# vgl-hub/teloscope

Hardware: AMD Instinct MI355X
Metric: Gbases/s scanned (whole node), 3 Gb FASTA TTAGGG w=1000 s=500 (higher is better)
Workload: dtype u8; 1 GPU; configs[1]: synthetic 3.00 Gb / 200 contigs, -c TTAGGG -p TTAGGG,TCAGGG,TGAGGG,TTGGGG -x 1 -w 1000 -s 500 -r -g -e -m -i, 124 patterns k=6; bases=3000000000, windows=6000095, matches=91510666, tiles=260970

## Files before the change

teloscope_amd/csrc/kernels.hip:

```cpp
#include <hip/hip_runtime.h>
#include <stdint.h>

#include <type_traits>

#include "ts_device.h"
#include "ts_internal.h"

#define set_prio(p) __builtin_amdgcn_s_setprio(p)
constexpr int kPrioPass = 3;
constexpr int kPrioAppend = 2;
constexpr int kPrioWindows = 2;

namespace {

typedef unsigned long long u64;
#define LDS __attribute__((address_space(3)))
typedef uint32_t u32x2 __attribute__((ext_vector_type(2)));
typedef LDS unsigned char lds_u8;
typedef LDS uint16_t lds_u16;
typedef LDS uint32_t lds_u32;

__device__ __forceinline__ lds_u16 *lds_at16(uint32_t addr) { return (lds_u16 *)(uintptr_t)addr; }
__device__ __forceinline__ lds_u8 *lds_at8(uint32_t addr) { return (lds_u8 *)(uintptr_t)addr; }

__host__ __device__ inline uint32_t align16(uint32_t x) { return (x + 15u) & ~15u; }

struct SliceLayout { uint32_t codes, rec, wacc, stage, park, bytes; };

__host__ __device__ inline SliceLayout slice_layout(const TsScanParams &P) {
    SliceLayout s;
    uint32_t o = 0;
    s.codes = o; o += align16((P.nch * 63u + 1u) * 8u);
    s.rec = o; o += (P.windows_on && P.nuc_on) ? align16((P.max_windows + P.halo_blocks) * 16u) : 0u;
    s.wacc = o; o += P.windows_on ? align16((P.max_windows + (P.acc_blocks ? P.halo_blocks : 0u)) * 8u * (P.acc_copies + (P.acc_blocks ? 1u : 0u))) : 0u;
    s.stage = o; o += (P.stage_cap + 64u) * (P.stage_u16 ? 2u : 4u);
    s.park = o; o += 32u;
    s.bytes = o;
    return s;
}

__host__ __device__ inline uint32_t queue_region(const TsScanParams &P) {
    const uint32_t a = TS_LIST * 2u;
    return (P.table_rows * 4u + P.fc_bytes + a - 1u) & ~(a - 1u);
}

__host__ __device__ inline uint32_t lds_total(const TsScanParams &P) {
    return queue_region(P) + P.waves_per_wg * (TS_LIST * 2u + slice_layout(P).bytes);
}

template <bool FC_BYTES, bool PAIR_BYTES, int WAVES_EU, bool EMIT, bool FAST>
__global__ __launch_bounds__(TS_MAX_WG_THREADS, WAVES_EU)
void ts_scan_tiles(const TsScanParams P) {
    const bool st16 = FAST ? true : P.stage_u16 != 0u;
    const bool accb = FAST ? true : P.acc_blocks != 0u;
    extern __shared__ __attribute__((aligned(16))) unsigned char lds_raw[];
    const uint32_t tid = threadIdx.x;
    const uint32_t lane = tid & 63u;
    const uint32_t wave = (uint32_t)__builtin_amdgcn_readfirstlane((int)(tid >> 6));

    const uint32_t table_bytes = P.table_rows * 4u + P.fc_bytes;
    {
        const uint4 *src = (const uint4 *)P.table;
        uint4 *dst = (uint4 *)lds_raw;
        const uint32_t n16 = table_bytes >> 4;
        for (uint32_t i = tid; i < n16; i += blockDim.x) dst[i] = src[i];
    }
    __syncthreads();

    const SliceLayout SL = slice_layout(P);
    lds_u8 *lds = (lds_u8 *)lds_raw;
    uint32_t qbase = queue_region(P) + wave * (TS_LIST * 2u);
    uint32_t qmask = TS_LIST * 2u - 2u;
    asm volatile("" : "+v"(qbase));
    asm volatile("" : "+s"(qmask));
    lds_u8 *slice = lds + queue_region(P) + P.waves_per_wg * (TS_LIST * 2u) + wave * SL.bytes;
    lds_u32 *codes = (lds_u32 *)(slice + SL.codes);
    lds_u32 *rec = (lds_u32 *)(slice + SL.rec);
    lds_u32 *stage = (lds_u32 *)(slice + SL.stage);
    LDS u64 *wacc = (LDS u64 *)(slice + SL.wacc);
    lds_u32 *park = (lds_u32 *)(slice + SL.park);
    const uint32_t acc_rows = P.max_windows + (accb ? P.halo_blocks : 0u);
    const uint32_t acc_off = (lane & (P.acc_copies - 1u)) * acc_rows;

    const uint32_t k = P.k;
    const uint32_t rowbits = 2u * (k + 1u) - 4u;
    const uint32_t kmask = (1u << (2u * k)) - 1u;
    const uint32_t pmask = (1u << (2u * (k + 1u))) - 1u;
    const lds_u32 *fc_table = (const lds_u32 *)(lds + P.table_rows * 4u);
    const lds_u8 *fc_bytes = (const lds_u8 *)fc_table;
    const uint32_t tab_base = (uint32_t)(uintptr_t)lds;
    if (PAIR_BYTES && (tab_base & pmask) != 0u) __builtin_trap();

    const uint32_t total_waves = gridDim.x * P.waves_per_wg;
    const uint32_t gw = blockIdx.x * P.waves_per_wg + wave;
    typedef const TsScanParams __attribute__((address_space(4))) *KernArgs;
    auto tail_params = [&]() -> KernArgs {
        KernArgs q = (KernArgs)__builtin_amdgcn_kernarg_segment_ptr();
        asm volatile("" : "+s"(q));
        return q;
    };
    uint32_t cursor = 0;
    if (EMIT) { park[4] = 0u; park[5] = 0u; }
    const uint32_t nwper = P.halo_blocks + 1u;

    typedef const TsTile __attribute__((address_space(4))) *ConstTiles;
    const ConstTiles const_tiles = (ConstTiles)(uintptr_t)P.tiles;
    uint4 n0 = make_uint4(0, 0, 0, 0), n1 = n0;
    uint32_t ticket = 0;
    const uint32_t ngroups = P.dynamic_tiles ? P.ticket_groups : 1u;
    const uint32_t group = blockIdx.x % ngroups;
    const uint32_t group_waves = ((gridDim.x - group + ngroups - 1u) / ngroups) * P.waves_per_wg;
    auto take_ticket = [&](KernArgs Q) -> uint32_t {
        const u64 a = (u64)(uintptr_t)(Q->tile_tickets + (Q->ticket_slot * Q->ticket_groups + group) * TS_TICKET_STRIDE);
        uint32_t lo = (uint32_t)a, hi = (uint32_t)(a >> 32);
        asm volatile("" : "+v"(lo), "+v"(hi));
        typedef __attribute__((address_space(1))) uint32_t *GlobalU32;
        return __hip_atomic_fetch_add((GlobalU32)(uintptr_t)(((u64)hi << 32) | lo), 1u, __ATOMIC_RELAXED, __HIP_MEMORY_SCOPE_AGENT);
    };
    if (P.dynamic_tiles && gw == 0 && lane < ngroups) P.tile_tickets[((1u - P.ticket_slot) * ngroups + lane) * TS_TICKET_STRIDE] = 0u;
    const uint32_t first_tile = P.dynamic_tiles ? group + ngroups * ((blockIdx.x / ngroups) * P.waves_per_wg + wave) : gw;
    if (first_tile < P.ntiles) {
        if (P.dynamic_tiles && lane == 0) ticket = take_ticket(tail_params());
        const unsigned char *ls = P.in + (const_tiles[first_tile].in_off & ~15ull) + lane * 32u;
        n0 = *(const uint4 *)ls; n1 = *(const uint4 *)(ls + 16);
    }
    for (uint32_t tile = first_tile, tile_next = 0; tile < P.ntiles; tile = tile_next) {
        struct { u64 in_off; uint32_t nrel, nwin, own_len; } T;
        {
            const ConstTiles q = const_tiles + tile;
            uint32_t lo = (uint32_t)q->in_off, hi = (uint32_t)(q->in_off >> 32), a = q->nrel, b = q->nwin, c = q->own_len;
            asm volatile("" : "+s"(lo), "+s"(hi), "+s"(a), "+s"(b), "+s"(c));
            T.in_off = ((u64)hi << 32) | lo; T.nrel = a; T.nwin = b; T.own_len = c;
        }
        const uint32_t sh = (uint32_t)(T.in_off & 15ull);
        const unsigned char *src = P.in + (T.in_off - sh);
        const uint32_t nblk = T.nwin + P.halo_blocks;
        const uint32_t span = nblk * P.s;
        const uint32_t xend = sh + T.nrel;
        uint32_t need = sh + (T.nrel < span + 16u ? T.nrel : span + 16u);
        uint32_t nch = (need + 16u + TS_CHUNK - 1u) / TS_CHUNK;
        if (nch > P.nch) nch = P.nch;
        nch = (uint32_t)__builtin_amdgcn_readfirstlane((int)nch);
        bool has_invalid = false;
        const uint32_t own_end = sh + T.own_len;
        uint32_t done = 0, ccan = 0, cfwd = 0;
        uint32_t flushed = 0;
        auto stage_at = [&](uint32_t i) -> uint32_t { return st16 ? (uint32_t)((lds_u16 *)stage)[i] : stage[i]; };
        auto flush_stage = [&]() {
            __builtin_amdgcn_wave_barrier();
            const uint32_t n = done - flushed;
            KernArgs Q = tail_params();
            const uint32_t cap = Q->region_cap;
            uint32_t *const wave_out = Q->matches_out + (u64)gw * cap;
            const bool rec16 = Q->rec16 != 0u;
            for (uint32_t i = lane; i < n; i += 64u) {
                const uint32_t o = cursor + flushed + i;
                if (o < cap) {
                    if (rec16) gstore_lo16((uint16_t *)Q->matches_out + (u64)gw * cap + o, stage_at(i));
                    else gstore(wave_out + o, stage_at(i));
                }
            }
            if (EMIT) park[5] = 1u;
            __builtin_amdgcn_s_waitcnt(0x0F70);
            __builtin_amdgcn_wave_barrier();
            flushed = done;
        };
        uint32_t tile_vis = 0;
        auto finish_records = [&]() {
            __builtin_amdgcn_wave_barrier();
            KernArgs Q = tail_params();
            const uint32_t cap = Q->region_cap;
            uint32_t *const wave_out = Q->matches_out + (u64)gw * cap;
            uint32_t ln = lane;
            asm volatile("" : "+v"(ln));
            uint32_t n = done - flushed;
            bool redo = false;
            if (EMIT) redo = __builtin_amdgcn_readfirstlane((int)park[5]) != 0;
            const bool rec16 = Q->rec16 != 0u;
            uint16_t *const wave_out16 = (uint16_t *)Q->matches_out + (u64)gw * cap;
            if (!EMIT || redo) {
                if (!EMIT && st16 && rec16 && cursor + flushed + n <= cap) {
                    const uint32_t n4 = n & ~3u;
                    uint16_t *const dst = wave_out16 + cursor + flushed;
                    for (uint32_t i = 4u * ln; i < n4; i += 256u) {
                        const u32x2 q = *(const LDS u32x2 *)((lds_u16 *)stage + i);
                        gstore_unaligned((unsigned char *)(dst + i), (u64)q.x | ((u64)q.y << 32));
                    }
                    if (ln < n - n4) gstore_lo16(dst + n4 + ln, stage_at(n4 + ln));
                } else
                for (uint32_t i = ln; i < n; i += 64u) {
                    const uint32_t o = cursor + flushed + i;
                    if (o < cap) {
                        if (rec16) gstore_lo16(wave_out16 + o, stage_at(i));
                        else gstore(wave_out + o, stage_at(i));
                    }
                }
                flushed = done;
                if (!EMIT) return;
                asm volatile("s_waitcnt vmcnt(0)" ::: "memory");
                park[5] = 0u;
                n = done;
            }
            const uint32_t base = redo ? 0u : flushed;
            uint32_t ch_first = 0, ch_last = 0, ch_cc = 0, ch_w1 = 0, vout = 0;
            const uint32_t vbase = (uint32_t)__builtin_amdgcn_readfirstlane((int)park[4]);
            typedef const uint32_t __attribute__((address_space(4))) *ConstU32;
            const uint32_t zone = ((ConstU32)(uintptr_t)Q->tile_zone)[tile];
            const uint32_t vis_cap = Q->vis_cap;
            const bool wide = FAST ? false : Q->vis_wide != 0u;
            void *const vis_out = Q->vis_out;
            const u64 vwave = (u64)gw * vis_cap;
            const uint32_t kdist = P.kdist;
            const bool rec_fit = cursor + base + n <= cap, vis_fit = vbase + n <= vis_cap;
            auto look = [&](const uint32_t r, const uint32_t nrow, const uint32_t i0, auto full_row) {
                constexpr bool FULL = decltype(full_row)::value;
                const uint32_t u = r >> 2;
                const u64 live_m = FULL ? ~0ull : low_bits(nrow);
                const u64 canm = ballot64((r & 1u) != 0u);
                if (i0 == 0u) ch_first = (uint32_t)__builtin_amdgcn_readfirstlane((int)u);
                {
                    u64 vm = canm;
                    if (zone != TS_ZONE_NONE) vm = live_m & (canm | ballot64(u < (zone & 0xFFFFu)) | ballot64(u >= (zone >> 16)));
                    if (vm != 0ull) {
                        const uint32_t at = vbase + vout + __builtin_amdgcn_mbcnt_hi((uint32_t)(vm >> 32), __builtin_amdgcn_mbcnt_lo((uint32_t)vm, 0u));
                        if (__builtin_amdgcn_inverse_ballot_w64(vm) && (vis_fit || at < vis_cap)) {
                            if (wide) gstore((uint32_t *)vis_out + (vwave + at), r);
                            else gstore((uint16_t *)vis_out + (vwave + at), (uint16_t)r);
                        }
                        vout += (uint32_t)__popcll(vm);
                    }
                }
                const uint32_t ncan = (uint32_t)__popcll(canm);
                const uint32_t t = ch_cc + ncan;
                if ((t | (~ch_w1 & TS_CHAIN_HEADS)) != 0u) {
                    const uint32_t below = lane_below(u, ch_last);
                    const u64 H = FULL ? ballot64(u - below > kdist) : live_m & ballot64(u - below > kdist);
                    if (__builtin_expect(t >= 4u, 0)) {
                        if (H != 0ull) {
                            const u64 ahead = ~H & (H - 1ull);
                            const uint32_t top_head = 63u - (uint32_t)__builtin_clzll(H);
                            const u64 below_top = low_bits(top_head);
                            const uint32_t carry = ch_cc + (uint32_t)__popcll(canm & ahead);
                            if (!(ch_w1 & TS_CHAIN_HEADS)) ch_w1 |= carry < 0x7FFFu ? carry : 0x7FFFu;
                            else if (carry >= 4u) ch_w1 |= TS_CHAIN_INNER;
                            if (__popcll(canm & ~ahead & below_top) >= 4) {
                                const u64 above = ln < 63u ? H >> (ln + 1u) : 0ull;
                                const uint32_t next = above ? ln + 1u + (uint32_t)__builtin_ctzll(above) : 64u;
                                const bool mine4 = __popcll(canm & low_bits(next) & ~low_bits(ln)) >= 4;
                                if (ballot64(((H >> ln) & 1ull) && ln != top_head && mine4) != 0ull) ch_w1 |= TS_CHAIN_INNER;
                            }
                            ch_w1 |= TS_CHAIN_HEADS;
                            ch_cc = (uint32_t)__popcll(canm & ~below_top);
                        } else {
                            ch_cc = t;
                        }
                    } else {
                        uint32_t tmp;
                        u64 m;
                        asm volatile("s_bitcmp1_b32 %[w1], 15\n\t"
                                     "s_cbranch_scc1 .Lts_cq%=\n\t"
                                     "s_cmp_eq_u64 %[H], 0\n\t"
                                     "s_cbranch_scc1 .Lts_cq%=\n\t"
                                     "s_ff1_i32_b64 %[tmp], %[H]\n\t"
                                     "s_lshl_b64 %[m], -1, %[tmp]\n\t"
                                     "s_andn2_b64 %[m], %[canm], %[m]\n\t"
                                     "s_bcnt1_i32_b64 %[tmp], %[m]\n\t"
                                     "s_add_i32 %[tmp], %[tmp], %[cc]\n\t"
                                     "s_or_b32 %[w1], %[w1], %[tmp]\n\t"
                                     "s_bitset1_b32 %[w1], 15\n"
                                     ".Lts_cq%=:\n\t"
                                     "s_flbit_i32_b64 %[tmp], %[H]\n\t"
                                     "s_xor_b32 %[tmp], %[tmp], 63\n\t"
                                     "s_lshl_b64 %[m], -1, %[tmp]\n\t"
                                     "s_and_b64 %[m], %[m], %[canm]\n\t"
                                     "s_bcnt1_i32_b64 %[tmp], %[m]\n\t"
                                     "s_cmp_lg_u64 %[H], 0\n\t"
                                     "s_cselect_b32 %[cc], %[tmp], %[t]"
                                     : [cc] "+s"(ch_cc), [w1] "+s"(ch_w1), [tmp] "=&s"(tmp), [m] "=&s"(m)
                                     : [H] "s"(H), [canm] "s"(canm), [t] "s"(t)
                                     : "scc");
                    }
                }
                ch_last = (uint32_t)__builtin_amdgcn_readlane((int)u, FULL ? 63 : (int)nrow - 1);
            };
            if (!redo) {
                const uint32_t nfull = n & ~63u;
                for (uint32_t i0 = 0; i0 < nfull; i0 += 64u) {
                    const uint32_t o = cursor + base + i0 + ln;
                    const uint32_t r = stage_at(i0 + ln);
                    auto put = [&]() { if (rec16) gstore_lo16(wave_out16 + o, r); else gstore(wave_out + o, r); };
                    if (rec_fit) put();
                    else if (o < cap) put();
                    look(r, 64u, i0, std::true_type{});
                }
                for (uint32_t i0 = nfull; i0 < n; i0 += 64u) {
                    const uint32_t nrow = n - i0 < 64u ? n - i0 : 64u;
                    const uint32_t o = cursor + base + i0 + ln;
                    uint32_t r = 0u;
                    if (ln < nrow) {
                        r = stage_at(i0 + ln);
                        if (o < cap) {
                            if (rec16) gstore_lo16(wave_out16 + o, r);
                            else gstore(wave_out + o, r);
                        }
                    }
                    look(r, nrow, i0, std::false_type{});
                }
            } else {
                for (uint32_t i0 = 0; i0 < n; i0 += 64u) {
                    const uint32_t nrow = n - i0 < 64u ? n - i0 : 64u;
                    const uint32_t o = cursor + base + i0 + ln;
                    uint32_t r = 0u;
                    if (ln < nrow && o < cap)
                        r = rec16 ? (uint32_t)__hip_atomic_load(wave_out16 + o, __ATOMIC_RELAXED, __HIP_MEMORY_SCOPE_AGENT)
                                  : __hip_atomic_load(wave_out + o, __ATOMIC_RELAXED, __HIP_MEMORY_SCOPE_AGENT);
                    look(r, nrow, i0, std::false_type{});
                }
            }
            flushed = done;
            const uint32_t z15 = ch_cc < 0x7FFFu ? ch_cc : 0x7FFFu;
            if (!(ch_w1 & TS_CHAIN_HEADS)) ch_w1 |= z15;
            const u64 voff = vwave + vbase;
            if (ln == 0u) gstore((uint4 *)&Q->tile_chain[4ull * tile], make_uint4((ch_first & 0xFFFFu) | (ch_last << 16), ch_w1 | (z15 << 16), (uint32_t)voff, (uint32_t)(voff >> 32)));
            tile_vis = vout;
            park[4] = vbase + vout;
        };
        if (P.windows_on)
            for (uint32_t it = lane; it < acc_rows * 2u * (P.acc_copies + (accb ? 1u : 0u)); it += 64u) ((lds_u32 *)wacc)[it] = 0u;

        uint32_t qhead = 0, qcount = 0;
        auto drain_queue = [&](const uint32_t threshold) {
            if (qcount >= threshold && qcount > 0u) set_prio(kPrioPass);
            while (qcount >= threshold && qcount > 0u) {
                const uint32_t n = qcount < 64u ? qcount : 64u;
                if (done - flushed + 64u > P.stage_cap) flush_stage();
                const bool live = lane < n;
                const uint32_t xp = live ? (uint32_t)*lds_at16(((qhead + lane * 2u) & qmask) | qbase) : 0u;
                const lds_u32 *cw = codes + __builtin_amdgcn_ubfe(xp, 4, 12);
                const uint32_t kw = __builtin_amdgcn_alignbit(cw[1], cw[0], (xp & 15u) * 2u);
                const uint32_t idx = kw & kmask;
                uint32_t fc;
                if (PAIR_BYTES) fc = __builtin_amdgcn_ubfe((uint32_t)*lds_at8(kw & pmask), 2, 2);
                else if (FC_BYTES) fc = fc_bytes[idx];
                else fc = (fc_table[idx >> 4] >> ((idx & 15u) << 1)) & 3u;
                const uint32_t u = xp - sh;
                uint32_t q = 0u, o = u;
                if (P.windows_on) {
                    uint32_t qs;
                    if (P.div_exact) {
                        q = __umul24(u, P.s_magic22) >> 22; qs = __umul24(q, P.s);
                    } else {
                        q = __umul24(u, P.s_inv) >> 16; qs = __umul24(q, P.s);
                        if (qs > u) { --q; qs -= P.s; }
                    }
                    o = u - qs;
                }
                u64 valid_m = low_bits(n) & ballot64(xp >= sh);
                if (P.straddle_fix) valid_m &= ~ballot64(o + k > P.s);
                const u64 bal = valid_m & ballot64(xp < own_end);
                const bool valid = __builtin_amdgcn_inverse_ballot_w64(valid_m), owned = __builtin_amdgcn_inverse_ballot_w64(bal);
                const uint32_t rank = __builtin_amdgcn_mbcnt_hi((uint32_t)(bal >> 32), __builtin_amdgcn_mbcnt_lo((uint32_t)bal, 0u));
                const uint32_t slot = owned ? (done - flushed) + rank : P.stage_cap + lane;
                const uint32_t record = (u << 2) | fc;
                if (st16) ((lds_u16 *)stage)[slot] = (uint16_t)record; else stage[slot] = record;
                done += (uint32_t)__popcll(bal);
                const u64 can_all = ballot64((fc & 1u) != 0u), fwd_all = ballot64((fc & 2u) != 0u);
                const bool is_can = __builtin_amdgcn_inverse_ballot_w64(can_all), is_fwd = __builtin_amdgcn_inverse_ballot_w64(fwd_all);
                const u64 canm = can_all & bal;
                ccan += (uint32_t)__popcll(canm);
                cfwd += (uint32_t)__popcll(fwd_all & bal);
                const u64 inc = (u64)(is_can ? 1u : 0x10000u) | ((u64)(is_fwd ? 1u : 0x10000u) << 32);
                if (P.windows_on && accb) {
                    if (valid && q < nblk) atomicAdd((unsigned long long *)(wacc + acc_off + q), inc);
                    const u64 over = valid_m & ballot64(o + k > P.s);
                    if (over != 0ull) {
                        if (__builtin_amdgcn_inverse_ballot_w64(over) && q < nblk) atomicAdd((unsigned long long *)(wacc + P.acc_copies * acc_rows + q), inc);
                    }
                } else if (P.windows_on) {
                    for (uint32_t j = 0; j < nwper; ++j) {
                        const uint32_t wi = q - j;
                        const bool in = valid && wi < T.nwin && o + k + j * P.s <= P.w;
                        if (in) atomicAdd((unsigned long long *)(wacc + acc_off + wi), inc);
                    }
                }
                qhead = (qhead + 2u * n) & (TS_LIST * 2u - 1u);
                qcount -= n;
            }
            set_prio(0);
            __builtin_amdgcn_wave_barrier();
        };

        auto scan_chunk = [&](const uint32_t cpos, const uint32_t ch, const uint4 v0, const uint4 v1) -> uint32_t {
            const uint32_t x[8] = {v0.x, v0.y, v0.z, v0.w, v1.x, v1.y, v1.z, v1.w};
            uint32_t t[8], e[8], bad = 0;
#pragma unroll
            for (int i = 0; i < 8; ++i) {
                t[i] = x[i] & 0x06060606u;
                e[i] = __builtin_amdgcn_perm(0xFF47FF54u, 0xFF43FF41u, t[i]);
                bad = __builtin_amdgcn_bitop3_b32(x[i], e[i], bad, 0xBE);
            }
            uint32_t wa = pack16(t), wb = pack16(t + 4);

            const uint32_t pos0 = cpos + lane * 32u;
            uint32_t inv = 0;
            const bool slow = __any((bad & P.fold_mask) != 0u) || (cpos + 2048u > xend);
            if (slow) {
                asm volatile("; non-ACGT bases or segment end in this chunk" ::: "memory");
                uint32_t b4[8];
#pragma unroll
                for (int i = 0; i < 8; ++i) {
                    const uint32_t d = (x[i] & P.fold_mask) ^ e[i];
                    const uint32_t nz = ((((d & 0x7F7F7F7Fu) + 0x7F7F7F7Fu) | d) & 0x80808080u) >> 7;
                    b4[i] = __builtin_amdgcn_udot4(nz, 0x08040201u, 0u, false);
                }
                inv = b4[0] | (b4[1] << 4) | (b4[2] << 8) | (b4[3] << 12) |
                      (b4[4] << 16) | (b4[5] << 20) | (b4[6] << 24) | (b4[7] << 28);
                uint32_t inside = inv;
                if (pos0 < sh) inside &= ~0u << (sh - pos0);
                if (pos0 + 32u > xend) {
                    const uint32_t nv = xend > pos0 ? xend - pos0 : 0u;
                    inside &= ~(~0u << nv);
                    inv |= ~0u << nv;
                }
                if (__any(inside != 0u)) has_invalid = true;
                wa = pack16(t); wb = pack16(t + 4);
            }

            const uint32_t nx = (uint32_t)__builtin_amdgcn_mov_dpp((int)wa, 0x130, 0xf, 0xf, false);

            uint32_t tmp[16], ent[16];
            const uint32_t xa = PAIR_BYTES ? __builtin_amdgcn_alignbit(wb, wa, 16) : 0u;
            const uint32_t xb = PAIR_BYTES ? __builtin_amdgcn_alignbit(nx, wb, 16) : 0u;
#pragma unroll
            for (int j = 0; j < 16; ++j) {
                if (PAIR_BYTES) {
                    tmp[j] = 0;
                    const uint32_t word = (j & 7) <= 4 ? (j < 8 ? wa : wb) : (j < 8 ? xa : xb);
                    const uint32_t bit = (j & 7) <= 4 ? 4 * (j & 7) : 4 * ((j & 7) - 4);
                    const uint32_t addr = __builtin_amdgcn_ubfe(word, bit, 2u * (k + 1u)) | tab_base;
                    asm volatile("ds_read_u8 %0, %1" : "=v"(ent[j]) : "v"(addr));
                    continue;
                }
                if (j < 8) tmp[j] = (j == 0) ? wa : __builtin_amdgcn_alignbit(wb, wa, 4 * j);
                else tmp[j] = (j == 8) ? wb : __builtin_amdgcn_alignbit(nx, wb, 4 * (j - 8));
                {
                    const uint32_t row = __builtin_amdgcn_ubfe(tmp[j], 4, rowbits);
                    const uint32_t addr = tab_base + (row << 2);
                    asm volatile("ds_read_b32 %0, %1" : "=v"(ent[j]) : "v"(addr));
                }
            }
            const uint32_t h = ch + lane;
            *(LDS u32x2 *)(codes + 2u * h) = (u32x2){wa, wb};

            uint32_t M32 = 0;
            asm volatile("s_waitcnt lgkmcnt(0)" ::: "memory");
            __builtin_amdgcn_sched_barrier(0);
#pragma unroll
            for (int j = 0; j < 16; ++j)
                M32 = __builtin_amdgcn_alignbit(PAIR_BYTES ? ent[j] : ent[j] >> ((tmp[j] << 1) & 31u), M32, 2);

            if (slow) {
                const uint32_t inv_next = (uint32_t)__builtin_amdgcn_mov_dpp((int)inv, 0x130, 0xf, 0xf, false);
                const u64 iv = (u64)inv | ((u64)inv_next << 32);
                uint32_t kb = 0;
                for (uint32_t i = 0; i < k; ++i) kb |= (uint32_t)(iv >> i);
                M32 &= ~kb;
            }

            if (lane == 63u) M32 = 0;
            return M32;
        };
        auto append_chunk = [&](const uint32_t M32, const uint32_t cpos, const uint32_t nm0, const uint32_t incl0, const uint32_t total0) {
            const uint32_t lbase = cpos + lane * 32u;
            constexpr uint32_t kGroup = TS_LIST / 32u;
            const bool dense = TS_LIST < TS_CHUNK && total0 > TS_LIST;
            const uint32_t ngroups = dense ? 64u / kGroup : 1u;
            for (uint32_t gi = 0; gi < ngroups; ++gi) {
                uint32_t m = M32, nm = nm0, incl = incl0, total = total0;
                if (dense) {
                    m = (lane / kGroup == gi) ? M32 : 0u;
                    nm = __popc(m);
                    incl = wave_scan_add(nm);
                    total = (uint32_t)__builtin_amdgcn_readlane((int)incl, 63);
                }
                drain_queue(qcount + total > TS_LIST ? 1u : 64u);
                uint32_t o = qhead + 2u * (qcount + incl - nm);
                while (m) {
                    *lds_at16((o & qmask) | qbase) = (uint16_t)(lbase + (uint32_t)__builtin_ctz(m));
                    o += 2u;
                    m &= m - 1u;
                }
                qcount += total;
                __builtin_amdgcn_wave_barrier();
            }
        };
        auto append_pair = [&](const uint32_t mA, const uint32_t cposA, const uint32_t mB, const uint32_t cposB) {
            if (!__any((mA | mB) != 0u)) return;
            set_prio(kPrioAppend);
            const uint32_t nA = __popc(mA), nB = __popc(mB);
            const uint32_t incl = wave_scan_add(nA | (nB << 16));
            const uint32_t tot = (uint32_t)__builtin_amdgcn_readlane((int)incl, 63);
            const uint32_t totA = tot & 0xFFFFu, totB = tot >> 16;
            if (totA + totB + 63u > TS_LIST) {
                asm volatile("; dense pair of chunks" ::: "memory");
                if (totA) append_chunk(mA, cposA, nA, incl & 0xFFFFu, totA);
                if (totB) append_chunk(mB, cposB, nB, incl >> 16, totB);
                set_prio(0);
                return;
            }
            drain_queue(64u);
            set_prio(kPrioAppend);
            uint32_t o = qhead + 2u * (qcount + (incl & 0xFFFFu) - nA), m = mA;
            uint32_t lbase = cposA + lane * 32u;
            while (m) {
                *lds_at16((o & qmask) | qbase) = (uint16_t)(lbase + (uint32_t)__builtin_ctz(m));
                o += 2u;
                m &= m - 1u;
            }
            o = qhead + 2u * (qcount + totA + (incl >> 16) - nB); m = mB;
            lbase = cposB + lane * 32u;
            while (m) {
                *lds_at16((o & qmask) | qbase) = (uint16_t)(lbase + (uint32_t)__builtin_ctz(m));
                o += 2u;
                m &= m - 1u;
            }
            qcount += totA + totB;
            set_prio(0);
            __builtin_amdgcn_wave_barrier();
        };
        {
            const uint32_t last_pos = (uint32_t)__builtin_amdgcn_readfirstlane((int)((nch - 1u) * TS_CHUNK));
            const unsigned char *lsrc = src + lane * 32u;
            uint4 a0 = n0, a1 = n1, b0, b1;
            uint32_t cpos = 0, ch = 0;
            for (uint32_t c = 0; c < nch; c += 2u) {
                const uint32_t p1 = cpos + TS_CHUNK < last_pos ? cpos + TS_CHUNK : last_pos;
                b0 = *(const uint4 *)(lsrc + p1);
                b1 = *(const uint4 *)(lsrc + p1 + 16);
                __builtin_amdgcn_sched_barrier(0);
                const uint32_t mA = scan_chunk(cpos, ch, a0, a1);
                uint32_t mB = 0u;
                const bool pair = c + 1u < nch;
                if (pair) {
                    const uint32_t p2 = cpos + 2u * TS_CHUNK < last_pos ? cpos + 2u * TS_CHUNK : last_pos;
                    a0 = *(const uint4 *)(lsrc + p2);
                    a1 = *(const uint4 *)(lsrc + p2 + 16);
                    __builtin_amdgcn_sched_barrier(0);
                    mB = scan_chunk(cpos + TS_CHUNK, ch + 63u, b0, b1);
                }
                append_pair(mA, cpos, mB, cpos + TS_CHUNK);
                cpos += 2u * TS_CHUNK; ch += 126u;
            }
        }
#define TS_REQUEST_NEXT_TILE()                                                                                                   \
        {                                                                                                                        \
                           \
            __builtin_amdgcn_s_waitcnt(0x0F70);                                                                                  \
            KernArgs Q = tail_params();                                                                                          \
            const bool dyn = Q->dynamic_tiles != 0u;                                                                             \
            tile_next = dyn ? group + Q->ticket_groups * (group_waves + (uint32_t)__builtin_amdgcn_readfirstlane((int)ticket))   \
                            : tile + total_waves;                                                                                \
            if (tile_next < P.ntiles) {                       \
                const unsigned char *ls = P.in + (const_tiles[tile_next].in_off & ~15ull) + lane * 32u;                          \
                n0 = *(const uint4 *)ls; n1 = *(const uint4 *)(ls + 16);                                                         \
                if (dyn && lane == 0) ticket = take_ticket(Q);                         \
            }                                                                                                                    \
        }
        if (!EMIT) TS_REQUEST_NEXT_TILE()
        drain_queue(1u);
        __builtin_amdgcn_wave_barrier();

        set_prio(kPrioWindows);
        if (!EMIT) finish_records();
        if (EMIT) TS_REQUEST_NEXT_TILE()
        if (P.windows_on) {
            auto count_piece = [&](uint32_t xs, uint32_t xe, uint32_t &nL, uint32_t &nH, uint32_t &nG) {
                const uint32_t d0 = xs >> 4, d1 = (xe - 1u) >> 4;
                const uint32_t m0 = ~0u << (2u * (xs & 15u));
                const uint32_t m1 = ~0u >> (2u * (15u - ((xe - 1u) & 15u)));
                auto add2 = [&](uint32_t wA, uint32_t wB) {
                    const uint32_t lo = (wA & 0x55555555u) | ((wB << 1) & 0xAAAAAAAAu);
                    const uint32_t hi = ((wA >> 1) & 0x55555555u) | (wB & 0xAAAAAAAAu);
                    nL += __popc(lo); nH += __popc(hi); nG += __popc(lo & hi);
                };
                uint32_t first = codes[d0] & m0, last = 0u;
                if (d1 == d0) first &= m1; else last = codes[d1] & m1;
                add2(first, last);
                uint32_t d = d0 + 1u;
                for (; d + 2u <= d1; d += 2u) add2(codes[d], codes[d + 1u]);
                if (d < d1) add2(codes[d], 0u);
            };
            auto count_piece_bytes = [&](uint32_t xs, uint32_t xe, uint32_t n[4]) {
                const uint32_t fold = P.fold_mask & 0xFFu;
                for (uint32_t x = xs; x < xe; ++x) {
                    const uint32_t c = (uint32_t)src[x] & fold;
                    n[0] += c == 0x41u; n[1] += c == 0x43u; n[2] += c == 0x47u; n[3] += c == 0x54u;
                }
            };
            const bool by_blocks = P.block_sums != 0u;
            if (P.nuc_on) {
                const uint32_t rows = by_blocks ? T.nwin + P.halo_blocks : T.nwin;
                const uint32_t len = by_blocks ? P.s : P.w;
                for (uint32_t it = lane; it < rows * 4u; it += 64u) rec[it] = 0u;
                uint32_t pshift = 0;
                while (pshift < 2u && (rows << (pshift + 1u)) <= 64u && (len >> (pshift + 1u)) >= 128u) ++pshift;
                const uint32_t piece = (len + (1u << pshift) - 1u) >> pshift;
                __builtin_amdgcn_wave_barrier();
                for (uint32_t it = lane; it < (rows << pshift); it += 64u) {
                    const uint32_t row = it >> pshift, part = it & ((1u << pshift) - 1u);
                    const uint32_t row_end = row * P.s + len < T.nrel ? row * P.s + len : T.nrel;
                    const uint32_t us = row * P.s + part * piece;
                    const uint32_t ue = us + piece < row_end ? us + piece : row_end;
                    if (us >= ue) continue;
                    uint32_t n[4] = {0u, 0u, 0u, 0u};
                    if (has_invalid) {
                        count_piece_bytes(sh + us, sh + ue, n);
                    } else {
                        uint32_t nL = 0, nH = 0, nG = 0;
                        count_piece(sh + us, sh + ue, nL, nH, nG);
                        n[0] = (ue - us) + nG - nL - nH; n[1] = nL - nG; n[2] = nG; n[3] = nH - nG;
                    }
                    LDS uint32_t *r4 = rec + row * 4u;
                    if (pshift == 0u) { r4[0] = n[0]; r4[1] = n[1]; r4[2] = n[2]; r4[3] = n[3]; }
                    else {
#pragma unroll
                        for (int f = 0; f < 4; ++f) (void)__hip_atomic_fetch_add(r4 + f, n[f], __ATOMIC_RELAXED, __HIP_MEMORY_SCOPE_WORKGROUP);
                    }
                }
            }
            __builtin_amdgcn_wave_barrier();

            auto window_fields = [&](uint32_t i) -> u64 {
                u64 a = 0;
                if (accb) {
                    for (uint32_t c = 0; c < P.acc_copies; ++c)
                        for (uint32_t j = 0; j < nwper; ++j) a += wacc[c * acc_rows + i + j];
                    a -= wacc[P.acc_copies * acc_rows + i + nwper - 1u];
                } else {
                    for (uint32_t c = 0; c < P.acc_copies; ++c) a += wacc[c * acc_rows + i];
                }
                return a;
            };
            if (EMIT && tail_params()->win_packed != nullptr) {
                KernArgs Q = tail_params();
                const u64 T_win_out = const_tiles[tile].win_out;
                if (T_win_out >= Q->win_pack_lo && T_win_out < Q->win_pack_hi) {
                    const uint32_t wb = Q->win_pack_bytes, B = Q->win_field_bits;
                    unsigned char *const dst0 = Q->win_packed + T_win_out * (u64)wb;
                    uint32_t ln = lane;
                    asm volatile("" : "+v"(ln));
                    const bool ten = B == 10u && P.nuc_on != 0u;
                    for (uint32_t i = ln; i < T.nwin; i += 64u) {
                        u64 lo = 0, hi = 0;
                        uint32_t at = 0;
                        auto put = [&](uint32_t v) {
                            lo |= at < 64u ? (u64)v << at : 0ull;
                            if (at + B > 64u) hi |= at >= 64u ? (u64)v << (at - 64u) : (u64)v >> (64u - at);
                            at += B;
                        };
                        uint4 v = make_uint4(0u, 0u, 0u, 0u);
                        if (P.nuc_on) {
                            const uint32_t nrow = by_blocks ? P.halo_blocks + 1u : 1u;
                            for (uint32_t j = 0; j < nrow; ++j) {
                                const LDS uint32_t *r4 = rec + (i + j) * 4u;
                                v.x += r4[0]; v.y += r4[1]; v.z += r4[2]; v.w += r4[3];
                            }
                        }
                        const u64 a = window_fields(i);
                        const uint32_t f4 = (uint32_t)a & 0xFFFFu, f5 = (uint32_t)a >> 16, f6 = (uint32_t)(a >> 32) & 0xFFFFu;
                        if (ten) {
                            const uint32_t w0 = v.x | (v.y << 10) | (v.z << 20) | (v.w << 30);
                            const uint32_t w1 = (v.w >> 2) | (f4 << 8) | (f5 << 18) | (f6 << 28);
                            lo = (u64)w0 | ((u64)w1 << 32);
                            hi = (u64)(f6 >> 4);
                        } else {
                            if (P.nuc_on) { put(v.x); put(v.y); put(v.z); put(v.w); }
                            put(f4); put(f5); put(f6);
                        }
                        unsigned char *d = dst0 + (u64)i * wb;
                        uint32_t b = 0;
                        if (wb >= 8u) { gstore_unaligned(d, lo); b = 8u; }
                        if (wb - b >= 4u) { const uint32_t x = b ? (uint32_t)hi : (uint32_t)lo; gstore_unaligned(d + b, x); b += 4u; }
                        for (; b < wb; ++b) gstore(d + b, (unsigned char)(b < 8u ? lo >> (8u * b) : hi >> (8u * (b - 8u))));
                    }
                }
            } else {
                uint4 *wout = (uint4 *)(tail_params()->windows_out + const_tiles[tile].win_out * 8ull);
                for (uint32_t it = lane; it < T.nwin * 2u; it += 64u) {
                    const uint32_t i = it >> 1;
                    uint4 v = make_uint4(0u, 0u, 0u, 0u);
                    if (!(it & 1u)) {
                        if (P.nuc_on) {
                            const uint32_t nrow = by_blocks ? P.halo_blocks + 1u : 1u;
                            for (uint32_t j = 0; j < nrow; ++j) {
                                const LDS uint32_t *r4 = rec + (i + j) * 4u;
                                v.x += r4[0]; v.y += r4[1]; v.z += r4[2]; v.w += r4[3];
                            }
                        }
                    } else {
                        const u64 a = window_fields(i);
                        v.x = ((uint32_t)a & 0xFFFFu) * k; v.y = ((uint32_t)a >> 16) * k;
                        v.z = ((uint32_t)(a >> 32) & 0xFFFFu) * k; v.w = (uint32_t)(a >> 48) * k;
                    }
                    gstore(wout + it, v);
                }
            }
        }

        if (EMIT) finish_records();
        {
            const uint32_t tcan = ccan, tfwd = cfwd;
            if (lane == 0) {
                KernArgs Q = tail_params();
                gstore((u64 *)&Q->tile_off[tile], (u64)gw * Q->region_cap + cursor);
                const uint32_t vout = EMIT ? tile_vis : 0u;
                gstore((uint4 *)&Q->tile_stats[4ull * tile], make_uint4(done, tcan, tfwd, vout));
            }
            cursor += done;
        }
        set_prio(0);
        __builtin_amdgcn_wave_barrier();
    }
    if (lane == 0) {
        KernArgs Q = tail_params();
        Q->wave_fill[gw] = cursor;
        if (EMIT) Q->wave_fill[total_waves + gw] = park[4];
    }
}

__global__ void ts_segment_summary(const uint32_t *tile_stats, const uint32_t *seg_first_tile,
                                   const uint64_t *seg_nwin, uint32_t nseg, u64 *out) {
    __shared__ u64 part[3][256];
    const uint32_t sidx = blockIdx.x;
    if (sidx >= nseg) return;
    const uint32_t t0 = seg_first_tile[sidx], t1 = seg_first_tile[sidx + 1];
    u64 nm = 0, nc = 0, nf = 0;
    for (uint32_t t = t0 + threadIdx.x; t < t1; t += blockDim.x) {
        const uint4 st = *(const uint4 *)&tile_stats[4ull * t];
        nm += st.x; nc += st.y; nf += st.z;
    }
    part[0][threadIdx.x] = nm; part[1][threadIdx.x] = nc; part[2][threadIdx.x] = nf;
    __syncthreads();
    for (uint32_t o = 128; o >= 1; o >>= 1) {
        if (threadIdx.x < o) {
            part[0][threadIdx.x] += part[0][threadIdx.x + o];
            part[1][threadIdx.x] += part[1][threadIdx.x + o];
            part[2][threadIdx.x] += part[2][threadIdx.x + o];
        }
        __syncthreads();
    }
    if (threadIdx.x == 0) {
        out[4ull * sidx + 0] = seg_nwin[sidx];
        out[4ull * sidx + 1] = part[0][0];
        out[4ull * sidx + 2] = part[1][0];
        out[4ull * sidx + 3] = part[2][0];
    }
}

__global__ void ts_compact_regions(const uint32_t *regions, const uint32_t *wave_fill, const u64 *wave_dense_base,
                                   uint32_t region_cap, uint32_t nwaves, uint32_t *dense, int rec16) {
    const uint32_t w = blockIdx.x;
    if (w >= nwaves) return;
    const uint32_t n = wave_fill[w] < region_cap ? wave_fill[w] : region_cap;
    uint32_t *dst = dense + wave_dense_base[w];
    if (rec16) { const uint16_t *src = (const uint16_t *)regions + (u64)w * region_cap; for (uint32_t i = threadIdx.x; i < n; i += blockDim.x) dst[i] = src[i]; }
    else { const uint32_t *src = regions + (u64)w * region_cap; for (uint32_t i = threadIdx.x; i < n; i += blockDim.x) dst[i] = src[i]; }
}

}

int ts_k_lds_bytes(const TsScanParams *p) { return (int)lds_total(*p); }

namespace {
template <bool EMIT>
const void *scan_variant_e(const TsScanParams *p) {
    const bool two = p->wgs_per_cu > 1u;
    if (p->pair_byte_table && p->fc_byte_table) {
        const bool fast = p->stage_u16 && (!p->windows_on || p->acc_blocks);
        if (fast) return two ? (const void *)ts_scan_tiles<true, true, 6, EMIT, true> : (const void *)ts_scan_tiles<true, true, 4, EMIT, true>;
        return two ? (const void *)ts_scan_tiles<true, true, 6, EMIT, false> : (const void *)ts_scan_tiles<true, true, 4, EMIT, false>;
    }
    if (two) return nullptr;
    if (p->fc_byte_table) return (const void *)ts_scan_tiles<true, false, 4, EMIT, false>;
    return (const void *)ts_scan_tiles<false, false, 4, EMIT, false>;
}
const void *scan_variant(const TsScanParams *p) { return p->emit ? scan_variant_e<true>(p) : scan_variant_e<false>(p); }
}

int ts_k_prepare(uint32_t lds_bytes) {
    const void *fns[] = {(const void *)ts_scan_tiles<true, true, 4, false, false>, (const void *)ts_scan_tiles<true, false, 4, false, false>,
                         (const void *)ts_scan_tiles<false, false, 4, false, false>, (const void *)ts_scan_tiles<true, true, 6, false, false>,
                         (const void *)ts_scan_tiles<true, true, 4, true, false>, (const void *)ts_scan_tiles<true, false, 4, true, false>,
                         (const void *)ts_scan_tiles<false, false, 4, true, false>, (const void *)ts_scan_tiles<true, true, 6, true, false>,
                         (const void *)ts_scan_tiles<true, true, 4, false, true>, (const void *)ts_scan_tiles<true, true, 6, false, true>,
                         (const void *)ts_scan_tiles<true, true, 4, true, true>, (const void *)ts_scan_tiles<true, true, 6, true, true>};
    const int limit = (int)(lds_bytes > 160u * 1024u ? lds_bytes : 160u * 1024u);
    for (const void *fn : fns) {
        int e = (int)hipFuncSetAttribute(fn, hipFuncAttributeMaxDynamicSharedMemorySize, limit);
        if (e) return e;
    }
    return 0;
}

int ts_k_launch_scan(const TsScanParams *p, uint32_t grid, uint32_t lds_bytes, void *stream) {
    const dim3 block(p->waves_per_wg * 64u);
    const void *fn = scan_variant(p);
    if (!fn) return (int)hipErrorInvalidConfiguration;
    void *args[] = {(void *)p};
    return (int)hipLaunchKernel(fn, dim3(grid), block, args, lds_bytes, (hipStream_t)stream);
}

int ts_k_launch_summary(const uint32_t *tile_stats, const uint32_t *seg_first_tile, const uint64_t *seg_nwin,
                        uint32_t nseg, unsigned long long *out, void *stream) {
    if (nseg == 0) return 0;
    hipLaunchKernelGGL(ts_segment_summary, dim3(nseg), dim3(256), 0, (hipStream_t)stream,
                       tile_stats, seg_first_tile, seg_nwin, nseg, out);
    return (int)hipGetLastError();
}

int ts_k_launch_compact(const uint32_t *regions, const uint32_t *wave_fill, const unsigned long long *wave_dense_base,
                        uint32_t region_cap, uint32_t nwaves, uint32_t *dense, int rec16, void *stream) {
    if (nwaves == 0) return 0;
    hipLaunchKernelGGL(ts_compact_regions, dim3(nwaves), dim3(256), 0, (hipStream_t)stream,
                       regions, wave_fill, wave_dense_base, region_cap, nwaves, dense, rec16);
    return (int)hipGetLastError();
}
```

Baseline: 4388 Gbases/s.

## Prefetch next tile descriptor during chunk loop and hold ticket pointers in registers

```diff
diff --git a/profiles/handover_stamps.py b/profiles/handover_stamps.py
--- /dev/null
+++ b/profiles/handover_stamps.py
@@ -0,0 +1,63 @@
+#!/usr/bin/env python3
+import ctypes as C
+import os
+import sys
+
+ROOT = os.path.dirname(os.path.dirname(os.path.abspath(__file__)))
+sys.path.insert(0, ROOT)
+os.environ.setdefault("TELOSCAN_LIB", os.path.join(ROOT, "teloscope_amd", "libteloscan_stamps.so"))
+import numpy as np
+import torch
+
+import bench
+import teloscope_amd as ta
+from teloscope_amd import _capi as K
+from teloscope_amd import distributed as D
+from teloscope_amd.cli import parse_cli, user_input
+
+NAMES = ["window phase's end -> next tile's top (tile directory, loop)",
+         "tile's top -> first chunk in registers (descriptor, setup, zeroing, first-chunk wait)",
+         "chunk loop",
+         "chunk loop's end -> next tile's loads issued (hand-over)",
+         "hand-over -> window phase's end (last passes, records, windows)"]
+ROWS = 8192
+
+n = int(sys.argv[1]) if len(sys.argv) > 1 else 20
+emit = int(sys.argv[2]) if len(sys.argv) > 2 else 0
+dev = torch.device("cuda", 0)
+tel = ta.Teloscope(user_input(parse_cli("x.fa " + os.environ.get("TS_FLAGS", bench.FLAGS)), device=0))
+lens = bench.contig_lengths(int(float(os.environ.get("TS_GBASES", "3.0")) * 1e9), 200, 42)
+L = K.lib()
+stamps = L.ts_k_handover_stamps
+stamps.argtypes = [C.c_void_p, C.c_uint32, C.c_int]
+stamps.restype = C.c_int
+plan = D.ShardPlan(tel, lens, world=1)
+buf = torch.zeros(int(plan.info.input_bytes), dtype=torch.uint8, device=dev)
+bench.fill_synthetic(buf, plan.segment_offsets(), lens, 42, dev)
+L.ts_batch_set_emit(plan.batch, emit)
+st = torch.cuda.Stream(device=dev)
+sp, dp = C.c_void_p(st.cuda_stream), C.c_void_p(buf.data_ptr())
+with torch.cuda.stream(st):
+    for _ in range(bench.SETTLE_LAUNCHES):
+        assert L.ts_batch_scan(plan.batch, dp, sp) == 0
+    torch.cuda.synchronize()
+    assert L.ts_batch_sync(plan.batch) == 0
+    assert stamps(None, 0, 1) == 0
+    e0, e1 = torch.cuda.Event(enable_timing=True), torch.cuda.Event(enable_timing=True)
+    e0.record(st)
+    for _ in range(n):
+        L.ts_batch_scan(plan.batch, dp, sp)
+    e1.record(st)
+    torch.cuda.synchronize()
+rows = np.zeros((ROWS, 8), dtype=np.uint64)
+assert stamps(rows.ctypes.data, ROWS, 0) == 0
+rows = rows[rows[:, 5] > 0].astype(np.float64)
+tiles = rows[:, 5].sum()
+total = rows[:, :5].sum()
+print("%s build with stamps: %d launches, %.4f ms per launch, %d waves, %.1f tiles per wave and launch, %.0f ticks per tile"
+      % ("emitting" if emit else "plain", n, e0.elapsed_time(e1) / n, len(rows), tiles / len(rows) / n, total / tiles))
+share = rows[:, :5] / rows[:, :5].sum(axis=1, keepdims=True)
+for i in (1, 2, 3, 4, 0):
+    print("  %5.2f %% of wave time (waves: min %5.2f, max %5.2f)  %8.1f ticks per tile   %s"
+          % (100.0 * rows[:, i].sum() / total, 100.0 * share[:, i].min(), 100.0 * share[:, i].max(), rows[:, i].sum() / tiles, NAMES[i]))
+plan.close()
diff --git a/profiles/isa_counts.py b/profiles/isa_counts.py
--- /dev/null
+++ b/profiles/isa_counts.py
@@ -0,0 +1,27 @@
+#!/usr/bin/env python3
+import re
+import sys
+
+src = sys.argv[1]
+prefix = sys.argv[2] if len(sys.argv) > 2 else None
+cur, out = None, {}
+for line in open(src):
+    m = re.match(r"^_ZN12_GLOBAL__N_113ts_scan_tilesI(\w+?)EEv12TsScanParams:", line)
+    if m:
+        cur = m.group(1)
+        out[cur] = []
+    if cur is not None:
+        out[cur].append(line)
+        if re.match(r"^\.Lfunc_end", line):
+            cur = None
+NAMES = ("FC_BYTES", "PAIR_BYTES", "WAVES_EU", "EMIT", "FAST")
+print("%-44s %6s %7s %9s %9s %10s %8s %8s %7s %5s" % ("variant", "lines", "s_load", "lgkmcnt0", "readlane", "writelane", "readfirst", "vmcnt0", "scratch", "flat"))
+for k, v in out.items():
+    t = "".join(v)
+    c = lambda p: len(re.findall(p, t))
+    args = re.findall(r"L[bi](\d+)E", k)
+    label = " ".join("%s=%s" % nv for nv in zip(NAMES, args))
+    print("%-44s %6d %7d %9d %9d %10d %8d %8d %7d %5d" % (label, len(v), c(r"\ts_load_"), c(r"s_waitcnt[^\n]*lgkmcnt\(0\)"), c(r"v_readlane"),
+                                                        c(r"v_writelane"), c(r"v_readfirstlane"), c(r"s_waitcnt vmcnt\(0\)"), c(r"\tscratch_"), c(r"\tflat_")))
+    if prefix:
+        open("%s_%s.s" % (prefix, k), "w").writelines(v)
diff --git a/teloscope_amd/csrc/kernels.hip b/teloscope_amd/csrc/kernels.hip
--- a/teloscope_amd/csrc/kernels.hip
+++ b/teloscope_amd/csrc/kernels.hip
@@ -10,6 +10,23 @@
 constexpr int kPrioPass = 3;
 constexpr int kPrioAppend = 2;
 constexpr int kPrioWindows = 2;
+
+#ifdef TS_HANDOVER_STAMPS
+#define TS_STAMP_WAVES 8192
+__device__ unsigned long long ts_handover_stamp_buf[TS_STAMP_WAVES * 8];
+#define TS_PARK_BYTES 64u
+#define TS_STAMP(i)                                                                                                              \
+        {                                                                                                                        \
+            __builtin_amdgcn_sched_barrier(0);                                                                                   \
+            const uint32_t now_ = (uint32_t)__builtin_amdgcn_s_memtime();               \
+            park[8 + (i)] += now_ - park[14];                                                                                    \
+            park[14] = now_;                                                                                                     \
+            __builtin_amdgcn_sched_barrier(0);                                                                                   \
+        }
+#else
+#define TS_PARK_BYTES 32u
+#define TS_STAMP(i)
+#endif
 
 namespace {
 
@@ -34,7 +51,7 @@
     s.rec = o; o += (P.windows_on && P.nuc_on) ? align16((P.max_windows + P.halo_blocks) * 16u) : 0u;
     s.wacc = o; o += P.windows_on ? align16((P.max_windows + (P.acc_blocks ? P.halo_blocks : 0u)) * 8u * (P.acc_copies + (P.acc_blocks ? 1u : 0u))) : 0u;
     s.stage = o; o += (P.stage_cap + 64u) * (P.stage_u16 ? 2u : 4u);
-    s.park = o; o += 32u;
+    s.park = o; o += TS_PARK_BYTES;
     s.bytes = o;
     return s;
 }
@@ -102,6 +119,10 @@
     uint32_t cursor = 0;
     if (EMIT) { park[4] = 0u; park[5] = 0u; }
     const uint32_t nwper = P.halo_blocks + 1u;
+#ifdef TS_HANDOVER_STAMPS
+    for (uint32_t i = 8u; i < 16u; ++i) park[i] = 0u;
+    park[14] = (uint32_t)__builtin_amdgcn_s_memtime();
+#endif
 
     typedef const TsTile __attribute__((address_space(4))) *ConstTiles;
     const ConstTiles const_tiles = (ConstTiles)(uintptr_t)P.tiles;
@@ -110,30 +131,75 @@
     const uint32_t ngroups = P.dynamic_tiles ? P.ticket_groups : 1u;
     const uint32_t group = blockIdx.x % ngroups;
     const uint32_t group_waves = ((gridDim.x - group + ngroups - 1u) / ngroups) * P.waves_per_wg;
-    auto take_ticket = [&](KernArgs Q) -> uint32_t {
-        const u64 a = (u64)(uintptr_t)(Q->tile_tickets + (Q->ticket_slot * Q->ticket_groups + group) * TS_TICKET_STRIDE);
-        uint32_t lo = (uint32_t)a, hi = (uint32_t)(a >> 32);
-        asm volatile("" : "+v"(lo), "+v"(hi));
+    constexpr bool HELD = FAST || WAVES_EU == 4;
+    uint32_t tk_lo = 0u, tk_hi = 0u;
+    if (HELD) {
+        if (P.dynamic_tiles && lane == 0u) {
+            const u64 a = (u64)(uintptr_t)(P.tile_tickets + (P.ticket_slot * P.ticket_groups + group) * TS_TICKET_STRIDE);
+            tk_lo = (uint32_t)a; tk_hi = (uint32_t)(a >> 32);
+        }
+        asm volatile("" : "+v"(tk_lo), "+v"(tk_hi));
+    }
+    uint32_t tk_base = 0u, tk_mul = 0u;
+    if (HELD) {
+        tk_base = P.dynamic_tiles ? group + ngroups * group_waves : gw;
+        tk_mul = P.dynamic_tiles ? ngroups : total_waves;
+        asm volatile("" : "+v"(tk_base), "+v"(tk_mul));
+    }
+    auto take_ticket = [&]() -> uint32_t {
         typedef __attribute__((address_space(1))) uint32_t *GlobalU32;
+        uint32_t lo = tk_lo, hi = tk_hi;
+        if (!HELD) {
+            KernArgs Q = tail_params();
+            const u64 a = (u64)(uintptr_t)(Q->tile_tickets + (Q->ticket_slot * Q->ticket_groups + group) * TS_TICKET_STRIDE);
+            lo = (uint32_t)a; hi = (uint32_t)(a >> 32);
+            asm volatile("" : "+v"(lo), "+v"(hi));
+        }
         return __hip_atomic_fetch_add((GlobalU32)(uintptr_t)(((u64)hi << 32) | lo), 1u, __ATOMIC_RELAXED, __HIP_MEMORY_SCOPE_AGENT);
     };
+    auto takes_ticket = [&]() -> bool { return HELD ? (tk_lo | tk_hi) != 0u : tail_params()->dynamic_tiles != 0u && lane == 0u; };
+    uint32_t in_lo = 0u, in_hi = 0u;
+    if (HELD) {
+        const u64 a = (u64)(uintptr_t)P.in + lane * 32u;
+        in_lo = (uint32_t)a; in_hi = (uint32_t)(a >> 32);
+        asm volatile("" : "+v"(in_lo), "+v"(in_hi));
+    }
+    typedef const __attribute__((address_space(1))) unsigned char *GlobalIn;
+    typedef uint32_t u32x4 __attribute__((ext_vector_type(4)));
+    auto load16 = [](GlobalIn p) -> uint4 {
+        const u32x4 v = *(const __attribute__((address_space(1))) u32x4 *)p;
+        return make_uint4(v.x, v.y, v.z, v.w);
+    };
+    auto in_lane = [&]() -> GlobalIn {
+        return HELD ? (GlobalIn)(uintptr_t)(((u64)in_hi << 32) | in_lo) : (GlobalIn)(uintptr_t)(P.in + lane * 32u);
+    };
+    uint32_t desc = 0u, vnext = ~0u;
+    auto load_descriptor = [&](const TsTile *tiles, uint32_t t) -> uint32_t {
+        typedef const __attribute__((address_space(1))) uint32_t *GlobalCU32;
+        return ((GlobalCU32)(uintptr_t)tiles)[8ull * t + (lane & 7u)];
+    };
+    auto desc_word = [&](int i) -> uint32_t { return (uint32_t)__builtin_amdgcn_readlane((int)desc, i); };
+    auto desc_in_off = [&]() -> u64 { return ((u64)desc_word(1) << 32) | desc_word(0); };
     if (P.dynamic_tiles && gw == 0 && lane < ngroups) P.tile_tickets[((1u - P.ticket_slot) * ngroups + lane) * TS_TICKET_STRIDE] = 0u;
-    const uint32_t first_tile = P.dynamic_tiles ? group + ngroups * ((blockIdx.x / ngroups) * P.waves_per_wg + wave) : gw;
+    uint32_t first_tile = P.dynamic_tiles ? group + ngroups * ((blockIdx.x / ngroups) * P.waves_per_wg + wave) : gw;
     if (first_tile < P.ntiles) {
-        if (P.dynamic_tiles && lane == 0) ticket = take_ticket(tail_params());
-        const unsigned char *ls = P.in + (const_tiles[first_tile].in_off & ~15ull) + lane * 32u;
-        n0 = *(const uint4 *)ls; n1 = *(const uint4 *)(ls + 16);
-    }
-    for (uint32_t tile = first_tile, tile_next = 0; tile < P.ntiles; tile = tile_next) {
+        if (takes_ticket()) ticket = take_ticket();
+        desc = load_descriptor(P.tiles, first_tile);
+        const GlobalIn ls = in_lane() + (desc_in_off() & ~15ull);
+        n0 = load16(ls); n1 = load16(ls + 16);
+    } else {
+        first_tile = ~0u;
+    }
+    for (uint32_t tile = first_tile, tile_next = ~0u; tile != ~0u; tile = tile_next) {
         struct { u64 in_off; uint32_t nrel, nwin, own_len; } T;
         {
-            const ConstTiles q = const_tiles + tile;
-            uint32_t lo = (uint32_t)q->in_off, hi = (uint32_t)(q->in_off >> 32), a = q->nrel, b = q->nwin, c = q->own_len;
+            uint32_t lo = desc_word(0), hi = desc_word(1), a = desc_word(4), b = desc_word(5), c = desc_word(6);
             asm volatile("" : "+s"(lo), "+s"(hi), "+s"(a), "+s"(b), "+s"(c));
             T.in_off = ((u64)hi << 32) | lo; T.nrel = a; T.nwin = b; T.own_len = c;
         }
+        TS_STAMP(0)
         const uint32_t sh = (uint32_t)(T.in_off & 15ull);
-        const unsigned char *src = P.in + (T.in_off - sh);
+        const u64 src_off = T.in_off - sh;
         const uint32_t nblk = T.nwin + P.halo_blocks;
         const uint32_t span = nblk * P.s;
         const uint32_t xend = sh + T.nrel;
@@ -530,41 +596,76 @@
         };
         {
             const uint32_t last_pos = (uint32_t)__builtin_amdgcn_readfirstlane((int)((nch - 1u) * TS_CHUNK));
-            const unsigned char *lsrc = src + lane * 32u;
+            const GlobalIn lsrc = in_lane() + src_off;
             uint4 a0 = n0, a1 = n1, b0, b1;
             uint32_t cpos = 0, ch = 0;
+            typedef const __attribute__((address_space(1))) uint32_t *GlobalCU32;
+            uint32_t dn_lo = 0u, dn_hi = 0u;
+            if (HELD) {
+                KernArgs Q = tail_params();
+                uint32_t nt = Q->ntiles;
+                u64 tiles = (u64)(uintptr_t)Q->tiles;
+                asm volatile("" : "+s"(nt), "+s"(tiles));
+                if ((tk_lo | tk_hi) == 0u) ticket += 1u;
+                const uint32_t tv = tk_base + tk_mul * ticket;
+                vnext = tv < nt ? tv : ~0u;
+                const uint32_t t = (uint32_t)__builtin_amdgcn_readfirstlane((int)tv);
+                const u64 a = tiles + 32ull * (t < nt ? t : nt - 1u) + 4u * (lane & 7u);
+                dn_lo = (uint32_t)a; dn_hi = (uint32_t)(a >> 32);
+                asm volatile("" : "+v"(dn_lo), "+v"(dn_hi));
+            }
             for (uint32_t c = 0; c < nch; c += 2u) {
                 const uint32_t p1 = cpos + TS_CHUNK < last_pos ? cpos + TS_CHUNK : last_pos;
-                b0 = *(const uint4 *)(lsrc + p1);
-                b1 = *(const uint4 *)(lsrc + p1 + 16);
+                b0 = load16(lsrc + p1);
+                b1 = load16(lsrc + p1 + 16);
+                if (HELD) desc = *(GlobalCU32)(uintptr_t)(((u64)dn_hi << 32) | dn_lo);
                 __builtin_amdgcn_sched_barrier(0);
+#ifdef TS_HANDOVER_STAMPS
+                if (c == 0u) { asm volatile("" :: "v"(a0.x), "v"(a1.x)); TS_STAMP(1) }
+#endif
                 const uint32_t mA = scan_chunk(cpos, ch, a0, a1);
                 uint32_t mB = 0u;
                 const bool pair = c + 1u < nch;
                 if (pair) {
                     const uint32_t p2 = cpos + 2u * TS_CHUNK < last_pos ? cpos + 2u * TS_CHUNK : last_pos;
-                    a0 = *(const uint4 *)(lsrc + p2);
-                    a1 = *(const uint4 *)(lsrc + p2 + 16);
+                    a0 = load16(lsrc + p2);
+                    a1 = load16(lsrc + p2 + 16);
                     __builtin_amdgcn_sched_barrier(0);
                     mB = scan_chunk(cpos + TS_CHUNK, ch + 63u, b0, b1);
                 }
+                if (!HELD && c == 0u) {
+                    KernArgs Q = tail_params();
+                    uint32_t nt = Q->ntiles, dyn = Q->dynamic_tiles, tg = Q->ticket_groups;
+                    u64 tiles = (u64)(uintptr_t)Q->tiles;
+                    asm volatile("" : "+s"(nt), "+s"(dyn), "+s"(tg), "+s"(tiles));
+                    const uint32_t t = dyn ? group + tg * (group_waves + (uint32_t)__builtin_amdgcn_readfirstlane((int)ticket)) : tile + total_waves;
+                    desc = load_descriptor((const TsTile *)(uintptr_t)tiles, t < nt ? t : nt - 1u);
+                }
                 append_pair(mA, cpos, mB, cpos + TS_CHUNK);
                 cpos += 2u * TS_CHUNK; ch += 126u;
             }
         }
+        TS_STAMP(2)
 #define TS_REQUEST_NEXT_TILE()                                                                                                   \
         {                                                                                                                        \
                            \
             __builtin_amdgcn_s_waitcnt(0x0F70);                                                                                  \
-            KernArgs Q = tail_params();                                                                                          \
-            const bool dyn = Q->dynamic_tiles != 0u;                                                                             \
-            tile_next = dyn ? group + Q->ticket_groups * (group_waves + (uint32_t)__builtin_amdgcn_readfirstlane((int)ticket))   \
-                            : tile + total_waves;                                                                                \
-            if (tile_next < P.ntiles) {                       \
-                const unsigned char *ls = P.in + (const_tiles[tile_next].in_off & ~15ull) + lane * 32u;                          \
-                n0 = *(const uint4 *)ls; n1 = *(const uint4 *)(ls + 16);                                                         \
-                if (dyn && lane == 0) ticket = take_ticket(Q);                         \
+                 \
+            if (HELD) {                                                                                                          \
+                tile_next = (uint32_t)__builtin_amdgcn_readfirstlane((int)vnext);                                                \
+            } else {                                       \
+                KernArgs Q = tail_params();                                                                                      \
+                const uint32_t nt = Q->ntiles, dyn = Q->dynamic_tiles, tg = Q->ticket_groups;                                    \
+                tile_next = dyn ? group + tg * (group_waves + (uint32_t)__builtin_amdgcn_readfirstlane((int)ticket))             \
+                                : tile + total_waves;                                                                            \
+                if (tile_next >= nt) tile_next = ~0u;                                                                            \
             }                                                                                                                    \
+            if (tile_next != ~0u) {                                    \
+                const GlobalIn ls = in_lane() + (desc_in_off() & ~15ull);                                                        \
+                n0 = load16(ls); n1 = load16(ls + 16);                                                                           \
+                if (takes_ticket()) ticket = take_ticket();                            \
+            }                                                                                                                    \
+            TS_STAMP(3)                                                                                                          \
         }
         if (!EMIT) TS_REQUEST_NEXT_TILE()
         drain_queue(1u);
@@ -592,6 +693,7 @@
             };
             auto count_piece_bytes = [&](uint32_t xs, uint32_t xe, uint32_t n[4]) {
                 const uint32_t fold = P.fold_mask & 0xFFu;
+                const unsigned char *const src = tail_params()->in + src_off;
                 for (uint32_t x = xs; x < xe; ++x) {
                     const uint32_t c = (uint32_t)src[x] & fold;
                     n[0] += c == 0x41u; n[1] += c == 0x43u; n[2] += c == 0x47u; n[3] += c == 0x54u;
@@ -708,6 +810,10 @@
         }
 
         if (EMIT) finish_records();
+        TS_STAMP(4)
+#ifdef TS_HANDOVER_STAMPS
+        park[13] += 1u;
+#endif
         {
             const uint32_t tcan = ccan, tfwd = cfwd;
             if (lane == 0) {
@@ -725,6 +831,10 @@
         KernArgs Q = tail_params();
         Q->wave_fill[gw] = cursor;
         if (EMIT) Q->wave_fill[total_waves + gw] = park[4];
+#ifdef TS_HANDOVER_STAMPS
+        if (gw < TS_STAMP_WAVES)
+            for (uint32_t i = 0; i < 6u; ++i) ts_handover_stamp_buf[8u * gw + i] += park[8u + i];
+#endif
     }
 }
 
@@ -770,6 +880,18 @@
 }
 
 int ts_k_lds_bytes(const TsScanParams *p) { return (int)lds_total(*p); }
+
+#ifdef TS_HANDOVER_STAMPS
+extern "C" int ts_k_handover_stamps(unsigned long long *dst, uint32_t rows, int reset) {
+    int e = (int)hipDeviceSynchronize();
+    const size_t n = (size_t)(rows < TS_STAMP_WAVES ? rows : TS_STAMP_WAVES) * 8u * sizeof(unsigned long long);
+    if (!e && dst) e = (int)hipMemcpyFromSymbol(dst, HIP_SYMBOL(ts_handover_stamp_buf), n, 0, hipMemcpyDeviceToHost);
+    void *sym = nullptr;
+    if (!e && reset) e = (int)hipGetSymbolAddress(&sym, HIP_SYMBOL(ts_handover_stamp_buf));
+    if (!e && reset) e = (int)hipMemset(sym, 0, sizeof(unsigned long long) * TS_STAMP_WAVES * 8u);
+    return e;
+}
+#endif
 
 namespace {
 template <bool EMIT>
```

Result: slower. 4158 Gbases/s (-5.3%).
